# mratsim/constantine

Hardware: NVIDIA H100
Metric: bls12_381_g1_msm_throughput (higher is better)
Workload: dtype u32

## Files before the change

constantine_b200/csrc/msm_affine.cuh:

```cuda
#pragma once
#include "ec.cuh"
#include "field_inv.cuh"

namespace b200 {

constexpr int AFF_MAX_LEVELS = 8;
constexpr uint32_t AFF_NONE = 0xFFFFFFFFu;

static __global__ void k_bucket_bounds(const uint32_t* __restrict__ keys, size_t n, uint32_t no_key, uint32_t* head, uint32_t* tail) {
  size_t q = (size_t)blockIdx.x * blockDim.x + threadIdx.x;
  if (q >= n) return;
  const uint32_t key = keys[q];
  if (key >= no_key) return;
  if (q == 0 || keys[q - 1] != key) head[key] = (uint32_t)q;
  if (q + 1 == n || keys[q + 1] != key) tail[key] = (uint32_t)(q + 1);
}

constexpr int SCAN_THREADS = 256, SCAN_PER_THREAD = 4, SCAN_ITEMS = SCAN_THREADS * SCAN_PER_THREAD;

B200_DEV uint32_t block_exclusive_scan(uint32_t v, uint32_t& total, uint32_t* smem ) {
  const unsigned lane = threadIdx.x & 31u, warp = threadIdx.x >> 5;
  uint32_t inc = v;
#pragma unroll
  for (int d = 1; d < 32; d <<= 1) {
    uint32_t t = __shfl_up_sync(0xFFFFFFFFu, inc, d);
    if (lane >= (unsigned)d) inc += t;
  }
  __syncthreads();
  if (lane == 31u) smem[warp] = inc;
  __syncthreads();
  uint32_t base = 0, tot = 0;
#pragma unroll
  for (int w = 0; w < SCAN_THREADS / 32; w++) {
    const uint32_t s = smem[w];
    if ((unsigned)w < warp) base += s;
    tot += s;
  }
  total = tot;
  return base + inc - v;
}

B200_DEV uint32_t level_count(uint32_t n, int r) { return (n + (1u << r) - 1u) >> r; }

static __global__ void __launch_bounds__(SCAN_THREADS) k_level_blocksums(const uint32_t* __restrict__ head, const uint32_t* __restrict__ tail,
                                                                          uint32_t nb, int L, uint32_t nblk, uint32_t* blocksum ) {
  __shared__ uint32_t sm[SCAN_THREADS / 32 + 1];
  const uint32_t b0 = blockIdx.x * SCAN_ITEMS + threadIdx.x * SCAN_PER_THREAD;
  uint32_t cnt[SCAN_PER_THREAD];
#pragma unroll
  for (int k = 0; k < SCAN_PER_THREAD; k++) cnt[k] = (b0 + k < nb) ? tail[b0 + k] - head[b0 + k] : 0u;
  for (int r = 0; r <= L; r++) {
    uint32_t s = 0;
#pragma unroll
    for (int k = 0; k < SCAN_PER_THREAD; k++) s += level_count(cnt[k], r);
    uint32_t tot;
    block_exclusive_scan(s, tot, sm);
    if (threadIdx.x == 0) blocksum[(size_t)r * nblk + blockIdx.x] = tot;
  }
}

static __global__ void __launch_bounds__(SCAN_THREADS) k_level_scan(uint32_t* blocksum, uint32_t nblk, int L, uint32_t nb, uint32_t* off) {
  __shared__ uint32_t sm[SCAN_THREADS / 32 + 1];
  for (int r = 0; r <= L; r++) {
    uint32_t carry = 0;
    for (uint32_t base = 0; base < nblk; base += SCAN_THREADS) {
      const uint32_t i = base + threadIdx.x;
      const uint32_t v = (i < nblk) ? blocksum[(size_t)r * nblk + i] : 0u;
      uint32_t tot;
      const uint32_t ex = block_exclusive_scan(v, tot, sm);
      if (i < nblk) blocksum[(size_t)r * nblk + i] = carry + ex;
      carry += tot;
    }
    if (threadIdx.x == 0) off[(size_t)r * (nb + 1) + nb] = carry;
  }
}

static __global__ void __launch_bounds__(SCAN_THREADS) k_level_offsets(const uint32_t* __restrict__ head, const uint32_t* __restrict__ tail,
                                                                        uint32_t nb, int L, uint32_t nblk, const uint32_t* __restrict__ blocksum,
                                                                        uint32_t* off) {
  __shared__ uint32_t sm[SCAN_THREADS / 32 + 1];
  const uint32_t b0 = blockIdx.x * SCAN_ITEMS + threadIdx.x * SCAN_PER_THREAD;
  uint32_t cnt[SCAN_PER_THREAD];
#pragma unroll
  for (int k = 0; k < SCAN_PER_THREAD; k++) cnt[k] = (b0 + k < nb) ? tail[b0 + k] - head[b0 + k] : 0u;
  for (int r = 0; r <= L; r++) {
    uint32_t c[SCAN_PER_THREAD], s = 0;
#pragma unroll
    for (int k = 0; k < SCAN_PER_THREAD; k++) { c[k] = level_count(cnt[k], r); s += c[k]; }
    uint32_t tot;
    uint32_t ex = block_exclusive_scan(s, tot, sm) + blocksum[(size_t)r * nblk + blockIdx.x];
#pragma unroll
    for (int k = 0; k < SCAN_PER_THREAD; k++) {
      if (b0 + k < nb) off[(size_t)r * (nb + 1) + b0 + k] = ex;
      ex += c[k];
    }
  }
}

struct AffinePlan {
  uint2* plan0;
  uint32_t* plan[AFF_MAX_LEVELS];
  uint32_t* surv_keys;
  uint32_t* surv_vals;
};

static __global__ void k_affine_plan(const uint32_t* __restrict__ keys, const uint32_t* __restrict__ vals, size_t n, uint32_t no_key,
                                     const uint32_t* __restrict__ head, const uint32_t* __restrict__ tail,
                                     const uint32_t* __restrict__ off, uint32_t nb, int L, AffinePlan P) {
  size_t q = (size_t)blockIdx.x * blockDim.x + threadIdx.x;
  if (q >= n) return;
  const uint32_t b = keys[q];
  if (b >= no_key) return;
  const uint32_t h = head[b], i = (uint32_t)q - h, cnt = tail[b] - h;
  const size_t stride = (size_t)nb + 1;
  for (int r = 0; r < L; r++) {
    if (i & ((2u << r) - 1u)) break;
    const uint32_t p = off[(size_t)(r + 1) * stride + b] + (i >> (r + 1));
    const uint32_t s = i >> r;
    const bool has2 = s + 1u < level_count(cnt, r);
    if (r == 0) P.plan0[p] = make_uint2(vals[q], has2 ? vals[q + 1] : AFF_NONE);
    else P.plan[r][p] = (off[(size_t)r * stride + b] + s) | (has2 ? 0x80000000u : 0u);
  }
  if ((i & ((1u << L) - 1u)) == 0u) {
    const uint32_t ps = off[(size_t)L * stride + b] + (i >> L);
    P.surv_keys[ps] = b;
    P.surv_vals[ps] = ps;
  }
}

template <class T>
B200_DEV Aff<T> load_affine_rw(const uint32_t* base, size_t idx) {
  const uint32_t* p = base + idx * (2 * T::WORDS);
  Aff<T> a;
  load_words_rw(a.x, p);
  load_words_rw(a.y, p + T::WORDS);
  return a;
}
template <class T>
B200_DEV void store_affine(uint32_t* base, size_t idx, const Aff<T>& a) {
  uint32_t* p = base + idx * (2 * T::WORDS);
  store_words(p, a.x);
  store_words(p + T::WORDS, a.y);
}

template <class T>
B200_DEV void scratch_store(uint4* scratch, size_t threads, size_t tid, uint32_t j, const T& v) {
  constexpr int V = T::WORDS / 4;
#pragma unroll
  for (int k = 0; k < V; k++) {
    uint4 w;
    w.x = v.word(4 * k + 0); w.y = v.word(4 * k + 1); w.z = v.word(4 * k + 2); w.w = v.word(4 * k + 3);
    scratch[((size_t)j * V + k) * threads + tid] = w;
  }
}
template <class T>
B200_DEV T scratch_load(const uint4* scratch, size_t threads, size_t tid, uint32_t j) {
  constexpr int V = T::WORDS / 4;
  T v;
#pragma unroll
  for (int k = 0; k < V; k++) {
    const uint4 w = scratch[((size_t)j * V + k) * threads + tid];
    v.set_word(4 * k + 0, w.x); v.set_word(4 * k + 1, w.y); v.set_word(4 * k + 2, w.z); v.set_word(4 * k + 3, w.w);
  }
  return v;
}

constexpr int PART_TILE = 1024, PART_THREADS = 256, PART_MAX = 8;

B200_DEV uint32_t pair_chunk(const uint2 task, uint32_t n_points, uint32_t P) {
  uint32_t idx = task.x & 0x7FFFFFFFu;
  if (task.y != AFF_NONE) { const uint32_t j = task.y & 0x7FFFFFFFu; if (j > idx) idx = j; }
  uint32_t q = (uint32_t)(((unsigned long long)idx * P) / n_points);
  return q < P ? q : P - 1u;
}

static __global__ void __launch_bounds__(PART_THREADS) k_part_count(const uint2* __restrict__ plan0, const uint32_t* __restrict__ total_ptr,
                                                                    uint32_t n_points, uint32_t P, uint32_t nblk, uint32_t* counts) {
  __shared__ uint32_t sm[PART_MAX];
  if (threadIdx.x < PART_MAX) sm[threadIdx.x] = 0;
  __syncthreads();
  const uint32_t total = *total_ptr;
  const uint32_t base = blockIdx.x * PART_TILE;
  uint32_t local[PART_MAX];
#pragma unroll
  for (int q = 0; q < PART_MAX; q++) local[q] = 0;
  for (uint32_t i = threadIdx.x; i < PART_TILE; i += PART_THREADS) {
    const uint32_t p = base + i;
    if (p < total) {
      const uint32_t q = pair_chunk(plan0[p], n_points, P);
#pragma unroll
      for (int k = 0; k < PART_MAX; k++) local[k] += (q == (uint32_t)k) ? 1u : 0u;
    }
  }
#pragma unroll
  for (int q = 0; q < PART_MAX; q++) {
    uint32_t v = local[q];
    for (int d = 16; d >= 1; d >>= 1) v += __shfl_xor_sync(0xFFFFFFFFu, v, d);
    if ((threadIdx.x & 31u) == 0 && v) atomicAdd(&sm[q], v);
  }
  __syncthreads();
  if (threadIdx.x < P) counts[threadIdx.x * nblk + blockIdx.x] = sm[threadIdx.x];
}

static __global__ void __launch_bounds__(SCAN_THREADS) k_part_scan(uint32_t* counts, uint32_t P, uint32_t nblk, uint32_t* starts) {
  __shared__ uint32_t sm[SCAN_THREADS / 32 + 1];
  uint32_t carry = 0;
  const uint32_t len = P * nblk;
  for (uint32_t base = 0; base < len; base += SCAN_THREADS) {
    const uint32_t i = base + threadIdx.x;
    const uint32_t v = (i < len) ? counts[i] : 0u;
    uint32_t tot;
    const uint32_t ex = block_exclusive_scan(v, tot, sm);
    if (i < len) {
      counts[i] = carry + ex;
      if (i % nblk == 0) starts[i / nblk] = carry + ex;
    }
    carry += tot;
  }
  if (threadIdx.x == 0) starts[P] = carry;
}

static __global__ void __launch_bounds__(PART_THREADS) k_part_scatter(const uint2* __restrict__ plan0, const uint32_t* __restrict__ total_ptr,
                                                                      uint32_t n_points, uint32_t P, uint32_t nblk,
                                                                      const uint32_t* __restrict__ offsets, uint32_t* perm) {
  __shared__ uint32_t warp_cnt[PART_THREADS / 32][PART_MAX];
  __shared__ uint32_t run_base[PART_MAX];
  const uint32_t total = *total_ptr;
  const unsigned lane = threadIdx.x & 31u, warp = threadIdx.x >> 5;
  if (threadIdx.x < PART_MAX) run_base[threadIdx.x] = (threadIdx.x < P) ? offsets[threadIdx.x * nblk + blockIdx.x] : 0u;
  __syncthreads();
  for (uint32_t round = 0; round < PART_TILE / PART_THREADS; round++) {
    const uint32_t p = blockIdx.x * PART_TILE + round * PART_THREADS + threadIdx.x;
    const bool live = p < total;
    const uint32_t q = live ? pair_chunk(plan0[p], n_points, P) : 0xFFFFFFFFu;
    uint32_t my_rank = 0;
    for (uint32_t k = 0; k < P; k++) {
      const unsigned m = __ballot_sync(0xFFFFFFFFu, q == k);
      if (q == k) my_rank = __popc(m & ((1u << lane) - 1u));
      if (lane == 0) warp_cnt[warp][k] = __popc(m);
    }
    __syncthreads();
    if (live) {
      uint32_t before = 0;
      for (unsigned w = 0; w < warp; w++) before += warp_cnt[w][q];
      perm[run_base[q] + before + my_rank] = p;
    }
    __syncthreads();
    if (threadIdx.x < P) {
      uint32_t tot = 0;
      for (unsigned w = 0; w < PART_THREADS / 32; w++) tot += warp_cnt[w][threadIdx.x];
      run_base[threadIdx.x] += tot;
    }
    __syncthreads();
  }
}

enum PairKind { PAIR_COPY1 = 0, PAIR_COPY2 = 1, PAIR_INF = 2, PAIR_ADD = 3, PAIR_DBL = 4 };

struct PairTask {
  uint32_t a, b;
};
template <bool FIRST>
B200_DEV PairTask load_task(const void* plan, size_t p) {
  PairTask t;
  if constexpr (FIRST) {
    const uint2 v = reinterpret_cast<const uint2*>(plan)[p];
    t.a = v.x; t.b = v.y;
  } else {
    const uint32_t v = reinterpret_cast<const uint32_t*>(plan)[p];
    t.a = v & 0x7FFFFFFFu;
    t.b = (v >> 31) ? t.a + 1u : AFF_NONE;
  }
  return t;
}
template <class T, bool FIRST>
B200_DEV T load_x(const uint32_t* src, uint32_t ref) {
  T x;
  if constexpr (FIRST) load_words(x, src + (size_t)(ref & 0x7FFFFFFFu) * (2 * T::WORDS));
  else load_words_rw(x, src + (size_t)ref * (2 * T::WORDS));
  return x;
}
template <class T, bool FIRST>
B200_DEV T load_y(const uint32_t* src, uint32_t ref, bool& is_inf_if_x_zero) {
  T y;
  if constexpr (FIRST) {
    load_words(y, src + (size_t)(ref & 0x7FFFFFFFu) * (2 * T::WORDS) + T::WORDS);
    is_inf_if_x_zero = y.is_zero();
    y.cneg((ref >> 31) != 0);
  } else {
    load_words_rw(y, src + (size_t)ref * (2 * T::WORDS) + T::WORDS);
    is_inf_if_x_zero = y.is_zero();
  }
  return y;
}

template <class T>
B200_DEV int classify_pair(bool single, const T& x1, const T& y1, bool inf1, const T& x2, const T& y2, bool inf2, T& den) {
  if (single) return PAIR_COPY1;
  if (inf1) return PAIR_COPY2;
  if (inf2) return PAIR_COPY1;
  den = x2 - x1;
  if (!den.is_zero()) return PAIR_ADD;
  if (!(y1 == y2) || y1.is_zero()) return PAIR_INF;
  den = y1.dbl();
  return PAIR_DBL;
}

#ifndef B200_AFF_THREADS
#define B200_AFF_THREADS 128
#endif
#ifndef B200_AFF_MIN_BLOCKS
#define B200_AFF_MIN_BLOCKS 4
#endif

B200_DEV void prefetch_l2(const void* p) { asm volatile("prefetch.global.L2 [%0];" ::"l"(p)); }
B200_DEV void prefetch_span(const void* p, int bytes) {
  prefetch_l2(p);
  prefetch_l2((const char*)p + bytes - 1);
}
template <class T, bool FIRST>
B200_DEV void prefetch_point(const uint32_t* src, uint32_t ref) {
  const uint32_t idx = FIRST ? (ref & 0x7FFFFFFFu) : ref;
  prefetch_span(src + (size_t)idx * (2 * T::WORDS), 2 * T::WORDS * 4);
}

template <class T, bool FIRST>
__global__ void __launch_bounds__(B200_AFF_THREADS, (T::WORDS <= 12) ? B200_AFF_MIN_BLOCKS : 1)
k_affine_pairs(const void* __restrict__ plan, const uint32_t* __restrict__ total_ptr, const uint32_t* src, uint32_t* dst, uint4* scratch,
               const uint32_t* __restrict__ perm = nullptr, const uint32_t* __restrict__ range = nullptr) {
  const size_t threads = (size_t)gridDim.x * blockDim.x;
  const size_t tid = (size_t)blockIdx.x * blockDim.x + threadIdx.x;
  const uint32_t range_begin = range ? range[0] : 0u;
  const uint32_t total = range ? range[1] - range[0] : *total_ptr;
  if (perm) perm += range_begin;
  const uint32_t M = (uint32_t)(((size_t)total + threads - 1) / threads);
  const unsigned lane = threadIdx.x & 31u;
  const size_t warp_base = (tid - lane) * (size_t)M;
  if (warp_base >= total) return;
  uint32_t cnt = 0;
  {
    const size_t first = warp_base + lane;
    if (first < total) {
      const size_t left = (size_t)total - first;
      cnt = (uint32_t)((left + 31) / 32);
      if (cnt > M) cnt = M;
    }
  }
  T run = T::one();
  {
    auto slot_of = [&](size_t t) -> size_t { return perm ? (size_t)perm[t] : t; };
    PairTask t_next = cnt ? load_task<FIRST>(plan, slot_of(warp_base + lane)) : PairTask{0u, AFF_NONE};
    T x1n = T::zero(), x2n = T::zero();
    if (cnt) {
      x1n = load_x<T, FIRST>(src, t_next.a);
      if (t_next.b != AFF_NONE) x2n = load_x<T, FIRST>(src, t_next.b);
    }
#pragma unroll 1
    for (uint32_t j = 0; j < cnt; j++) {
      const PairTask t = t_next;
      const T x1 = x1n, x2 = x2n;
      if (j + 1 < cnt) {
        t_next = load_task<FIRST>(plan, slot_of(warp_base + lane + 32u * (size_t)(j + 1)));
        x1n = load_x<T, FIRST>(src, t_next.a);
        if (t_next.b != AFF_NONE) x2n = load_x<T, FIRST>(src, t_next.b);
      }
      const bool single = t.b == AFF_NONE;
      T den = x2 - x1;
      bool contributes = !single;
      if (!single && (den.is_zero() || x1.is_zero() || x2.is_zero())) {
        bool z1, z2;
        const T y1 = load_y<T, FIRST>(src, t.a, z1), y2 = load_y<T, FIRST>(src, t.b, z2);
        const int kind = classify_pair(false, x1, y1, z1 && x1.is_zero(), x2, y2, z2 && x2.is_zero(), den);
        contributes = kind >= PAIR_ADD;
      }
      if (contributes) run = run.mul_u(den);
      scratch_store(scratch, threads, tid, j, run);
    }
  }
  T inv = fe_inverse(run);
  auto slot_of2 = [&](size_t t) -> size_t { return perm ? (size_t)perm[t] : t; };
  size_t p_prev = cnt ? slot_of2(warp_base + lane + 32u * (size_t)(cnt - 1)) : 0;
  PairTask t_prev = cnt ? load_task<FIRST>(plan, p_prev) : PairTask{0u, AFF_NONE};
#pragma unroll 1
  for (uint32_t jj = cnt; jj > 0; jj--) {
    const uint32_t j = jj - 1;
    const size_t p = p_prev;
    const PairTask t = t_prev;
    if (j > 0) {
      p_prev = slot_of2(warp_base + lane + 32u * (size_t)(j - 1));
      t_prev = load_task<FIRST>(plan, p_prev);
      prefetch_point<T, FIRST>(src, t_prev.a);
      if (t_prev.b != AFF_NONE) prefetch_point<T, FIRST>(src, t_prev.b);
      if (j > 1) {
        constexpr int V = T::WORDS / 4;
#pragma unroll
        for (int k = 0; k < V; k++) prefetch_l2(scratch + ((size_t)(j - 2) * V + k) * threads + tid);
      }
    }
    const bool single = t.b == AFF_NONE;
    Aff<T> P1, P2;
    bool z1 = false, z2 = false;
    P1.x = load_x<T, FIRST>(src, t.a);
    P1.y = load_y<T, FIRST>(src, t.a, z1);
    if (!single) {
      P2.x = load_x<T, FIRST>(src, t.b);
      P2.y = load_y<T, FIRST>(src, t.b, z2);
    } else {
      P2.x = T::zero(); P2.y = T::zero();
    }
    T den;
    const int kind = classify_pair(single, P1.x, P1.y, z1 && P1.x.is_zero(), P2.x, P2.y, z2 && P2.x.is_zero(), den);
    Aff<T> R;
    if (kind < PAIR_ADD) {
      if (kind == PAIR_COPY1) R = P1;
      else if (kind == PAIR_COPY2) R = P2;
      else { R.x = T::zero(); R.y = T::zero(); }
    } else {
      T inv_den = inv;
      if (j > 0) inv_den = inv.mul_u(scratch_load<T>(scratch, threads, tid, j - 1));
      inv = inv.mul_u(den);
      T num;
      if (kind == PAIR_ADD) num = P2.y - P1.y;
      else { const T xx = P1.x.sqr(); num = xx.dbl() + xx; }
      const T lam = num.mul_u(inv_den);
      R.x = lam.sqr_u() - P1.x - P2.x;
      R.y = lam.mul_u(P1.x - R.x) - P1.y;
    }
    store_affine(dst, p, R);
  }
}

#ifndef B200_AFF_WS_CONSUMERS
#define B200_AFF_WS_CONSUMERS 8
#endif
#ifndef B200_AFF_WS_STAGES
#define B200_AFF_WS_STAGES 2
#endif
constexpr int AFF_WS_CONSUMERS = B200_AFF_WS_CONSUMERS;
constexpr int AFF_WS_THREADS = 32 * (AFF_WS_CONSUMERS + 1);

template <class T>
struct AffRing {
  static constexpr bool USED = T::WORDS <= 12;
  static constexpr int V = T::WORDS / 4;
  static constexpr int S2 = B200_AFF_WS_STAGES;
  static constexpr int ROWS = S2 * 5 * V;
  static constexpr int S1 = ROWS / (2 * V);
  static constexpr size_t BYTES = (size_t)AFF_WS_CONSUMERS * ROWS * 32 * 16;
};

B200_DEV uint32_t smem_addr(const void* p) { return (uint32_t)__cvta_generic_to_shared(p); }
B200_DEV void mbar_init(uint64_t* b, uint32_t count) { asm volatile("mbarrier.init.shared::cta.b64 [%0], %1;" ::"r"(smem_addr(b)), "r"(count) : "memory"); }
B200_DEV void mbar_arrive(uint64_t* b) { asm volatile("mbarrier.arrive.shared::cta.b64 _, [%0];" ::"r"(smem_addr(b)) : "memory"); }
B200_DEV void mbar_wait(uint64_t* b, uint32_t parity) {
  asm volatile(
      "{\n\t.reg .pred P1;\n"
      "WAIT:\n\t"
      "mbarrier.try_wait.parity.shared::cta.b64 P1, [%0], %1;\n\t"
      "@!P1 bra WAIT;\n\t}" ::"r"(smem_addr(b)),
      "r"(parity)
      : "memory");
}
B200_DEV void cp_async_arrive(uint64_t* b) { asm volatile("cp.async.mbarrier.arrive.noinc.shared::cta.b64 [%0];" ::"r"(smem_addr(b)) : "memory"); }
B200_DEV void cp_async16(void* s, const void* g) { asm volatile("cp.async.cg.shared.global [%0], [%1], 16;" ::"r"(smem_addr(s)), "l"(g) : "memory"); }

template <class T>
B200_DEV void ring_fetch(uint4* ring, int row, unsigned lane, const uint32_t* g) {
#pragma unroll
  for (int k = 0; k < T::WORDS / 4; k++) cp_async16(ring + (row + k) * 32 + lane, g + 4 * k);
}
template <class T>
B200_DEV T ring_load(const uint4* ring, int row, unsigned lane) {
  T v;
#pragma unroll
  for (int k = 0; k < T::WORDS / 4; k++) {
    const uint4 w = ring[(row + k) * 32 + lane];
    v.set_word(4 * k + 0, w.x); v.set_word(4 * k + 1, w.y); v.set_word(4 * k + 2, w.z); v.set_word(4 * k + 3, w.w);
  }
  return v;
}

template <class T, bool FIRST>
__global__ void __launch_bounds__(AFF_WS_THREADS, 1)
k_affine_pairs_ws(const void* __restrict__ plan, const uint32_t* __restrict__ total_ptr, const uint32_t* src, uint32_t* dst, uint4* scratch,
                  const uint32_t* __restrict__ perm = nullptr, const uint32_t* __restrict__ range = nullptr) {
  using RG = AffRing<T>;
  constexpr int V = RG::V, NC = AFF_WS_CONSUMERS, S1 = RG::S1, S2 = RG::S2;
  extern __shared__ __align__(16) unsigned char aff_ring_raw[];
  __shared__ uint64_t full1[NC][S1], empty1[NC][S1], full2[NC][S2], empty2[NC][S2], drained[NC];
  __shared__ uint32_t s_task[NC][S1][3][32];
  const unsigned lane = threadIdx.x & 31u, warp = threadIdx.x >> 5;
  if (threadIdx.x == 0) {
    for (int w = 0; w < NC; w++) {
      for (int s = 0; s < S1; s++) { mbar_init(&full1[w][s], 64); mbar_init(&empty1[w][s], 32); }
      for (int s = 0; s < S2; s++) { mbar_init(&full2[w][s], 64); mbar_init(&empty2[w][s], 32); }
      mbar_init(&drained[w], 32);
    }
  }
  __syncthreads();
  const size_t threads = (size_t)gridDim.x * NC * 32;
  const uint32_t range_begin = range ? range[0] : 0u;
  const uint32_t total = range ? range[1] - range[0] : *total_ptr;
  if (perm) perm += range_begin;
  const uint32_t M = (uint32_t)(((size_t)total + threads - 1) / threads);
  auto count_of = [&](size_t tid) -> uint32_t {
    const size_t first = (tid & ~(size_t)31) * M + (tid & 31u);
    if (first >= total) return 0u;
    const uint32_t c = (uint32_t)(((size_t)total - first + 31) / 32);
    return c < M ? c : M;
  };
  auto slot_at = [&](size_t tid, uint32_t j) -> size_t {
    const size_t t = (tid & ~(size_t)31) * M + (tid & 31u) + 32u * (size_t)j;
    return perm ? (size_t)perm[t] : t;
  };
  uint4* const ring_base = reinterpret_cast<uint4*>(aff_ring_raw);

  if (warp == NC) {
    uint32_t n[NC], cnt[NC];
#pragma unroll
    for (int w = 0; w < NC; w++) {
      const size_t tid = ((size_t)blockIdx.x * NC + w) * 32 + lane;
      n[w] = count_of(tid - lane);
      cnt[w] = count_of(tid);
    }
    auto tid_of = [&](int w) { return ((size_t)blockIdx.x * NC + w) * 32 + lane; };
    auto src_of = [&](uint32_t ref) { return src + (size_t)(FIRST ? (ref & 0x7FFFFFFFu) : ref) * (2 * T::WORDS); };
    uint32_t ta[NC], tb[NC], tp[NC];
    auto fetch_task = [&](int w, uint32_t j) {
      const size_t p = slot_at(tid_of(w), j);
      const PairTask t = load_task<FIRST>(plan, p);
      ta[w] = t.a; tb[w] = t.b; tp[w] = (uint32_t)p;
    };
#pragma unroll
    for (int w = 0; w < NC; w++) if (cnt[w]) fetch_task(w, 0);
#pragma unroll 1
    for (uint32_t j = 0; j < n[0]; j++) {
      uint32_t ca[NC], cb[NC];
#pragma unroll
      for (int w = 0; w < NC; w++) { ca[w] = ta[w]; cb[w] = tb[w]; }
#pragma unroll
      for (int w = 0; w < NC; w++) if (j + 1 < cnt[w]) fetch_task(w, j + 1);
#pragma unroll
      for (int w = 0; w < NC; w++) {
        if (j >= n[w]) continue;
        const int s = (int)(j % S1);
        mbar_wait(&empty1[w][s], ((j / S1) & 1u) ^ 1u);
        uint4* ring = ring_base + (size_t)w * RG::ROWS * 32;
        if (j < cnt[w]) {
          s_task[w][s][0][lane] = ca[w];
          s_task[w][s][1][lane] = cb[w];
          ring_fetch<T>(ring, s * 2 * V, lane, src_of(ca[w]));
          if (cb[w] != AFF_NONE) ring_fetch<T>(ring, s * 2 * V + V, lane, src_of(cb[w]));
        }
        cp_async_arrive(&full1[w][s]);
        mbar_arrive(&full1[w][s]);
      }
    }
#pragma unroll
    for (int w = 0; w < NC; w++) if (n[w] && n[w] - 1 < cnt[w]) fetch_task(w, n[w] - 1);
#pragma unroll 1
    for (uint32_t jj = 0; jj < n[0]; jj++) {
      uint32_t ca[NC], cb[NC], cp[NC];
#pragma unroll
      for (int w = 0; w < NC; w++) { ca[w] = ta[w]; cb[w] = tb[w]; cp[w] = tp[w]; }
#pragma unroll
      for (int w = 0; w < NC; w++) if (jj + 1 < n[w] && n[w] - 2 - jj < cnt[w]) fetch_task(w, n[w] - 2 - jj);
#pragma unroll
      for (int w = 0; w < NC; w++) {
        if (jj >= n[w]) continue;
        if (jj == 0) mbar_wait(&drained[w], 0);
        const uint32_t j = n[w] - 1 - jj;
        const int s = (int)(jj % S2);
        mbar_wait(&empty2[w][s], ((jj / S2) & 1u) ^ 1u);
        uint4* ring = ring_base + (size_t)w * RG::ROWS * 32;
        if (j < cnt[w]) {
          s_task[w][s][0][lane] = ca[w];
          s_task[w][s][1][lane] = cb[w];
          s_task[w][s][2][lane] = cp[w];
          const int row = s * 5 * V;
          ring_fetch<T>(ring, row, lane, src_of(ca[w]));
          ring_fetch<T>(ring, row + V, lane, src_of(ca[w]) + T::WORDS);
          if (cb[w] != AFF_NONE) {
            ring_fetch<T>(ring, row + 2 * V, lane, src_of(cb[w]));
            ring_fetch<T>(ring, row + 3 * V, lane, src_of(cb[w]) + T::WORDS);
          }
          if (j > 0) {
#pragma unroll
            for (int k = 0; k < V; k++)
              cp_async16(ring + (row + 4 * V + k) * 32 + lane, scratch + ((size_t)(j - 1) * V + k) * threads + tid_of(w));
          }
        }
        cp_async_arrive(&full2[w][s]);
        mbar_arrive(&full2[w][s]);
      }
    }
    asm volatile("cp.async.wait_all;" ::: "memory");
    return;
  }

  const size_t tid = ((size_t)blockIdx.x * NC + warp) * 32 + lane;
  const uint32_t n = count_of(tid - lane), cnt = count_of(tid);
  if (n == 0) return;
  const uint4* ring = ring_base + (size_t)warp * RG::ROWS * 32;
  T run = T::one();
#pragma unroll 1
  for (uint32_t j = 0; j < n; j++) {
    const int s = (int)(j % S1);
    mbar_wait(&full1[warp][s], (j / S1) & 1u);
    const uint32_t a = s_task[warp][s][0][lane], b = s_task[warp][s][1][lane];
    const T x1 = ring_load<T>(ring, s * 2 * V, lane), x2 = ring_load<T>(ring, s * 2 * V + V, lane);
    mbar_arrive(&empty1[warp][s]);
    if (j >= cnt) continue;
    const bool single = b == AFF_NONE;
    T den = x2 - x1;
    bool contributes = !single;
    if (!single && (den.is_zero() || x1.is_zero() || x2.is_zero())) {
      bool z1, z2;
      const T y1 = load_y<T, FIRST>(src, a, z1), y2 = load_y<T, FIRST>(src, b, z2);
      const int kind = classify_pair(false, x1, y1, z1 && x1.is_zero(), x2, y2, z2 && x2.is_zero(), den);
      contributes = kind >= PAIR_ADD;
    }
    if (contributes) run = run.mul_u(den);
    scratch_store(scratch, threads, tid, j, run);
  }
  mbar_arrive(&drained[warp]);
  T inv = fe_inverse(run);
#pragma unroll 1
  for (uint32_t jj = 0; jj < n; jj++) {
    const uint32_t j = n - 1 - jj;
    const int s = (int)(jj % S2);
    mbar_wait(&full2[warp][s], (jj / S2) & 1u);
    const int row = s * 5 * V;
    const uint32_t a = s_task[warp][s][0][lane], b = s_task[warp][s][1][lane], p = s_task[warp][s][2][lane];
    const bool single = b == AFF_NONE;
    Aff<T> P1, P2;
    P1.x = ring_load<T>(ring, row, lane);
    P1.y = ring_load<T>(ring, row + V, lane);
    P2.x = single ? T::zero() : ring_load<T>(ring, row + 2 * V, lane);
    P2.y = single ? T::zero() : ring_load<T>(ring, row + 3 * V, lane);
    const T pre = ring_load<T>(ring, row + 4 * V, lane);
    mbar_arrive(&empty2[warp][s]);
    if (j >= cnt) continue;
    const bool z1 = P1.y.is_zero(), z2 = P2.y.is_zero();
    if constexpr (FIRST) {
      P1.y.cneg((a >> 31) != 0);
      if (!single) P2.y.cneg((b >> 31) != 0);
    }
    T den;
    const int kind = classify_pair(single, P1.x, P1.y, z1 && P1.x.is_zero(), P2.x, P2.y, z2 && P2.x.is_zero(), den);
    Aff<T> R;
    if (kind < PAIR_ADD) {
      if (kind == PAIR_COPY1) R = P1;
      else if (kind == PAIR_COPY2) R = P2;
      else { R.x = T::zero(); R.y = T::zero(); }
    } else {
      T inv_den = inv;
      if (j > 0) inv_den = inv.mul_u(pre);
      inv = inv.mul_u(den);
      T num;
      if (kind == PAIR_ADD) num = P2.y - P1.y;
      else { const T xx = P1.x.sqr(); num = xx.dbl() + xx; }
      const T lam = num.mul_u(inv_den);
      R.x = lam.sqr_u() - P1.x - P2.x;
      R.y = lam.mul_u(P1.x - R.x) - P1.y;
    }
    store_affine(dst, p, R);
  }
}

template <class T>
constexpr int affine_pairs_slot_threads() { return AffRing<T>::USED ? 32 * AFF_WS_CONSUMERS : B200_AFF_THREADS; }

template <class T>
cudaError_t affine_pairs_blocks_per_sm(int* bps) {
  int b1 = 0, b2 = 0;
  cudaError_t e;
  if constexpr (AffRing<T>::USED) {
    constexpr int bytes = (int)AffRing<T>::BYTES;
    if ((e = cudaFuncSetAttribute(k_affine_pairs_ws<T, true>, cudaFuncAttributeMaxDynamicSharedMemorySize, bytes)) != cudaSuccess) return e;
    if ((e = cudaFuncSetAttribute(k_affine_pairs_ws<T, false>, cudaFuncAttributeMaxDynamicSharedMemorySize, bytes)) != cudaSuccess) return e;
    if ((e = cudaOccupancyMaxActiveBlocksPerMultiprocessor(&b1, k_affine_pairs_ws<T, true>, AFF_WS_THREADS, bytes)) != cudaSuccess) return e;
    if ((e = cudaOccupancyMaxActiveBlocksPerMultiprocessor(&b2, k_affine_pairs_ws<T, false>, AFF_WS_THREADS, bytes)) != cudaSuccess) return e;
  } else {
    if ((e = cudaOccupancyMaxActiveBlocksPerMultiprocessor(&b1, k_affine_pairs<T, true>, B200_AFF_THREADS, 0)) != cudaSuccess) return e;
    if ((e = cudaOccupancyMaxActiveBlocksPerMultiprocessor(&b2, k_affine_pairs<T, false>, B200_AFF_THREADS, 0)) != cudaSuccess) return e;
  }
  *bps = b2 < b1 ? b2 : b1;
  return cudaSuccess;
}

template <class T, bool FIRST>
void launch_affine_pairs(unsigned grid, cudaStream_t s, const void* plan, const uint32_t* total_ptr, const uint32_t* src, uint32_t* dst, uint4* scratch,
                         const uint32_t* perm = nullptr, const uint32_t* range = nullptr) {
  if constexpr (AffRing<T>::USED)
    k_affine_pairs_ws<T, FIRST><<<grid, AFF_WS_THREADS, AffRing<T>::BYTES, s>>>(plan, total_ptr, src, dst, scratch, perm, range);
  else
    k_affine_pairs<T, FIRST><<<grid, B200_AFF_THREADS, 0, s>>>(plan, total_ptr, src, dst, scratch, perm, range);
}

}
```

Measured before the change: 108.5.

## Split warp-specialized affine kernel into four producers and twelve consumers with setmaxnreg

Restructures the warp-specialized affine pair kernel from eight consumer warps fed by one producer warp into twelve consumers fed by four producer warps, each producer serving three consumers. setmaxnreg moves registers from the producers (32) to the consumers (160) so the consumers' field arithmetic has more register room. Task prefetch is interleaved with issuing fetches per consumer. The plan kernel is also rewritten to compute the level count with ffs and to preload offsets and values before the loop. The change depends on setmaxnreg behavior and carries a risk of spills if consumers need more than 160 registers.

```diff
diff --git a/constantine_b200/csrc/msm_affine.cuh b/constantine_b200/csrc/msm_affine.cuh
--- a/constantine_b200/csrc/msm_affine.cuh
+++ b/constantine_b200/csrc/msm_affine.cuh
@@ -113,16 +113,27 @@
   if (b >= no_key) return;
   const uint32_t h = head[b], i = (uint32_t)q - h, cnt = tail[b] - h;
   const size_t stride = (size_t)nb + 1;
-  for (int r = 0; r < L; r++) {
-    if (i & ((2u << r) - 1u)) break;
-    const uint32_t p = off[(size_t)(r + 1) * stride + b] + (i >> (r + 1));
+  const int lv = i ? min(__ffs((int)i) - 1, L) : L;
+  uint32_t o[AFF_MAX_LEVELS + 1];
+#pragma unroll
+  for (int r = 1; r <= AFF_MAX_LEVELS; r++) if (r <= lv) o[r] = off[(size_t)r * stride + b];
+  const uint32_t o_surv = lv == L ? off[(size_t)L * stride + b] : 0u;
+  uint32_t v0 = 0, v1 = AFF_NONE;
+  if (lv >= 1) {
+    v0 = vals[q];
+    if (i + 1u < cnt) v1 = vals[q + 1];
+  }
+#pragma unroll
+  for (int r = 0; r < AFF_MAX_LEVELS; r++) {
+    if (r >= lv) break;
+    const uint32_t p = o[r + 1] + (i >> (r + 1));
     const uint32_t s = i >> r;
     const bool has2 = s + 1u < level_count(cnt, r);
-    if (r == 0) P.plan0[p] = make_uint2(vals[q], has2 ? vals[q + 1] : AFF_NONE);
-    else P.plan[r][p] = (off[(size_t)r * stride + b] + s) | (has2 ? 0x80000000u : 0u);
-  }
-  if ((i & ((1u << L) - 1u)) == 0u) {
-    const uint32_t ps = off[(size_t)L * stride + b] + (i >> L);
+    if (r == 0) P.plan0[p] = make_uint2(v0, v1);
+    else P.plan[r][p] = (o[r] + s) | (has2 ? 0x80000000u : 0u);
+  }
+  if (lv == L) {
+    const uint32_t ps = o_surv + (i >> L);
     P.surv_keys[ps] = b;
     P.surv_vals[ps] = ps;
   }
@@ -430,14 +441,18 @@
   }
 }
 
-#ifndef B200_AFF_WS_CONSUMERS
-#define B200_AFF_WS_CONSUMERS 8
-#endif
 #ifndef B200_AFF_WS_STAGES
 #define B200_AFF_WS_STAGES 2
 #endif
-constexpr int AFF_WS_CONSUMERS = B200_AFF_WS_CONSUMERS;
-constexpr int AFF_WS_THREADS = 32 * (AFF_WS_CONSUMERS + 1);
+constexpr int AFF_WS_CONSUMERS = 12;
+constexpr int AFF_WS_PRODUCERS = 4;
+constexpr int AFF_WS_FEEDS = AFF_WS_CONSUMERS / AFF_WS_PRODUCERS;
+constexpr int AFF_WS_THREADS = 32 * (AFF_WS_CONSUMERS + AFF_WS_PRODUCERS);
+constexpr int AFF_WS_CONSUMER_REGS = 160, AFF_WS_PRODUCER_REGS = 32;
+static_assert(AFF_WS_CONSUMERS % 4 == 0 && AFF_WS_PRODUCERS == 4, "setmaxnreg acts on whole warpgroups");
+static_assert(32 * (AFF_WS_CONSUMERS * AFF_WS_CONSUMER_REGS + AFF_WS_PRODUCERS * AFF_WS_PRODUCER_REGS) == 65536 &&
+                  65536 / AFF_WS_THREADS == 128,
+              "the register split must fill exactly the registers the launch gives the block");
 
 template <class T>
 struct AffRing {
@@ -463,6 +478,10 @@
 }
 B200_DEV void cp_async_arrive(uint64_t* b) { asm volatile("cp.async.mbarrier.arrive.noinc.shared::cta.b64 [%0];" ::"r"(smem_addr(b)) : "memory"); }
 B200_DEV void cp_async16(void* s, const void* g) { asm volatile("cp.async.cg.shared.global [%0], [%1], 16;" ::"r"(smem_addr(s)), "l"(g) : "memory"); }
+template <int R>
+B200_DEV void setmaxnreg_inc() { asm volatile("setmaxnreg.inc.sync.aligned.u32 %0;" ::"n"(R)); }
+template <int R>
+B200_DEV void setmaxnreg_dec() { asm volatile("setmaxnreg.dec.sync.aligned.u32 %0;" ::"n"(R)); }
 
 template <class T>
 B200_DEV void ring_fetch(uint4* ring, int row, unsigned lane, const uint32_t* g) {
@@ -485,7 +504,7 @@
 k_affine_pairs_ws(const void* __restrict__ plan, const uint32_t* __restrict__ total_ptr, const uint32_t* src, uint32_t* dst, uint4* scratch,
                   const uint32_t* __restrict__ perm = nullptr, const uint32_t* __restrict__ range = nullptr) {
   using RG = AffRing<T>;
-  constexpr int V = RG::V, NC = AFF_WS_CONSUMERS, S1 = RG::S1, S2 = RG::S2;
+  constexpr int V = RG::V, NC = AFF_WS_CONSUMERS, F = AFF_WS_FEEDS, S1 = RG::S1, S2 = RG::S2;
   extern __shared__ __align__(16) unsigned char aff_ring_raw[];
   __shared__ uint64_t full1[NC][S1], empty1[NC][S1], full2[NC][S2], empty2[NC][S2], drained[NC];
   __shared__ uint32_t s_task[NC][S1][3][32];
@@ -509,95 +528,90 @@
     const uint32_t c = (uint32_t)(((size_t)total - first + 31) / 32);
     return c < M ? c : M;
   };
-  auto slot_at = [&](size_t tid, uint32_t j) -> size_t {
-    const size_t t = (tid & ~(size_t)31) * M + (tid & 31u) + 32u * (size_t)j;
-    return perm ? (size_t)perm[t] : t;
-  };
   uint4* const ring_base = reinterpret_cast<uint4*>(aff_ring_raw);
 
-  if (warp == NC) {
-    uint32_t n[NC], cnt[NC];
-#pragma unroll
-    for (int w = 0; w < NC; w++) {
-      const size_t tid = ((size_t)blockIdx.x * NC + w) * 32 + lane;
-      n[w] = count_of(tid - lane);
-      cnt[w] = count_of(tid);
-    }
-    auto tid_of = [&](int w) { return ((size_t)blockIdx.x * NC + w) * 32 + lane; };
+  if (warp >= NC) {
+    setmaxnreg_dec<AFF_WS_PRODUCER_REGS>();
+    const int w0 = (int)(warp - NC) * F;
+    const uint32_t tid0 = ((uint32_t)blockIdx.x * NC + w0) * 32 + lane;
+    auto first = [&](int i) { return (tid0 + 32u * i - lane) * M + lane; };
+    auto has_slot = [&](int i, uint32_t j) { return j < M && first(i) + 32u * j < total; };
+    auto rounds = [&](int i) -> uint32_t {
+      const uint32_t b = first(i) - lane;
+      return b < total ? min((total - b - 1) / 32 + 1, M) : 0u;
+    };
     auto src_of = [&](uint32_t ref) { return src + (size_t)(FIRST ? (ref & 0x7FFFFFFFu) : ref) * (2 * T::WORDS); };
-    uint32_t ta[NC], tb[NC], tp[NC];
-    auto fetch_task = [&](int w, uint32_t j) {
-      const size_t p = slot_at(tid_of(w), j);
-      const PairTask t = load_task<FIRST>(plan, p);
-      ta[w] = t.a; tb[w] = t.b; tp[w] = (uint32_t)p;
+    auto slot = [&](int i, uint32_t j) { const uint32_t t = first(i) + 32u * j; return perm ? perm[t] : t; };
+    uint32_t ta[F], tb[F];
+    auto fetch_task = [&](int i, uint32_t j) {
+      const PairTask tk = load_task<FIRST>(plan, slot(i, j));
+      ta[i] = tk.a; tb[i] = tk.b;
     };
 #pragma unroll
-    for (int w = 0; w < NC; w++) if (cnt[w]) fetch_task(w, 0);
+    for (int i = 0; i < F; i++) if (has_slot(i, 0)) fetch_task(i, 0);
 #pragma unroll 1
-    for (uint32_t j = 0; j < n[0]; j++) {
-      uint32_t ca[NC], cb[NC];
-#pragma unroll
-      for (int w = 0; w < NC; w++) { ca[w] = ta[w]; cb[w] = tb[w]; }
-#pragma unroll
-      for (int w = 0; w < NC; w++) if (j + 1 < cnt[w]) fetch_task(w, j + 1);
-#pragma unroll
-      for (int w = 0; w < NC; w++) {
-        if (j >= n[w]) continue;
-        const int s = (int)(j % S1);
+    for (uint32_t j = 0; j < rounds(0); j++) {
+#pragma unroll
+      for (int i = 0; i < F; i++) {
+        if (j >= rounds(i)) continue;
+        const int w = w0 + i, s = (int)(j % S1);
         mbar_wait(&empty1[w][s], ((j / S1) & 1u) ^ 1u);
         uint4* ring = ring_base + (size_t)w * RG::ROWS * 32;
-        if (j < cnt[w]) {
-          s_task[w][s][0][lane] = ca[w];
-          s_task[w][s][1][lane] = cb[w];
-          ring_fetch<T>(ring, s * 2 * V, lane, src_of(ca[w]));
-          if (cb[w] != AFF_NONE) ring_fetch<T>(ring, s * 2 * V + V, lane, src_of(cb[w]));
+        if (has_slot(i, j)) {
+          s_task[w][s][0][lane] = ta[i];
+          s_task[w][s][1][lane] = tb[i];
+          ring_fetch<T>(ring, s * 2 * V, lane, src_of(ta[i]));
+          if (tb[i] != AFF_NONE) ring_fetch<T>(ring, s * 2 * V + V, lane, src_of(tb[i]));
         }
         cp_async_arrive(&full1[w][s]);
         mbar_arrive(&full1[w][s]);
+        if (has_slot(i, j + 1)) fetch_task(i, j + 1);
       }
     }
 #pragma unroll
-    for (int w = 0; w < NC; w++) if (n[w] && n[w] - 1 < cnt[w]) fetch_task(w, n[w] - 1);
+    for (int i = 0; i < F; i++) {
+      const uint32_t r = rounds(i);
+      if (r && has_slot(i, r - 1)) fetch_task(i, r - 1);
+    }
 #pragma unroll 1
-    for (uint32_t jj = 0; jj < n[0]; jj++) {
-      uint32_t ca[NC], cb[NC], cp[NC];
-#pragma unroll
-      for (int w = 0; w < NC; w++) { ca[w] = ta[w]; cb[w] = tb[w]; cp[w] = tp[w]; }
-#pragma unroll
-      for (int w = 0; w < NC; w++) if (jj + 1 < n[w] && n[w] - 2 - jj < cnt[w]) fetch_task(w, n[w] - 2 - jj);
-#pragma unroll
-      for (int w = 0; w < NC; w++) {
-        if (jj >= n[w]) continue;
+    for (uint32_t jj = 0; jj < rounds(0); jj++) {
+#pragma unroll
+      for (int i = 0; i < F; i++) {
+        const uint32_t r = rounds(i);
+        if (jj >= r) continue;
+        const int w = w0 + i;
         if (jj == 0) mbar_wait(&drained[w], 0);
-        const uint32_t j = n[w] - 1 - jj;
+        const uint32_t j = r - 1 - jj;
         const int s = (int)(jj % S2);
         mbar_wait(&empty2[w][s], ((jj / S2) & 1u) ^ 1u);
         uint4* ring = ring_base + (size_t)w * RG::ROWS * 32;
-        if (j < cnt[w]) {
-          s_task[w][s][0][lane] = ca[w];
-          s_task[w][s][1][lane] = cb[w];
-          s_task[w][s][2][lane] = cp[w];
+        if (has_slot(i, j)) {
+          s_task[w][s][0][lane] = ta[i];
+          s_task[w][s][1][lane] = tb[i];
+          s_task[w][s][2][lane] = slot(i, j);
           const int row = s * 5 * V;
-          ring_fetch<T>(ring, row, lane, src_of(ca[w]));
-          ring_fetch<T>(ring, row + V, lane, src_of(ca[w]) + T::WORDS);
-          if (cb[w] != AFF_NONE) {
-            ring_fetch<T>(ring, row + 2 * V, lane, src_of(cb[w]));
-            ring_fetch<T>(ring, row + 3 * V, lane, src_of(cb[w]) + T::WORDS);
+          ring_fetch<T>(ring, row, lane, src_of(ta[i]));
+          ring_fetch<T>(ring, row + V, lane, src_of(ta[i]) + T::WORDS);
+          if (tb[i] != AFF_NONE) {
+            ring_fetch<T>(ring, row + 2 * V, lane, src_of(tb[i]));
+            ring_fetch<T>(ring, row + 3 * V, lane, src_of(tb[i]) + T::WORDS);
           }
           if (j > 0) {
 #pragma unroll
             for (int k = 0; k < V; k++)
-              cp_async16(ring + (row + 4 * V + k) * 32 + lane, scratch + ((size_t)(j - 1) * V + k) * threads + tid_of(w));
+              cp_async16(ring + (row + 4 * V + k) * 32 + lane, scratch + ((size_t)(j - 1) * V + k) * threads + (tid0 + 32u * i));
           }
         }
         cp_async_arrive(&full2[w][s]);
         mbar_arrive(&full2[w][s]);
+        if (j > 0 && has_slot(i, j - 1)) fetch_task(i, j - 1);
       }
     }
     asm volatile("cp.async.wait_all;" ::: "memory");
     return;
   }
 
+  setmaxnreg_inc<AFF_WS_CONSUMER_REGS>();
   const size_t tid = ((size_t)blockIdx.x * NC + warp) * 32 + lane;
   const uint32_t n = count_of(tid - lane), cnt = count_of(tid);
   if (n == 0) return;
```

After: 113.0 (median of 6 runs). 1.04x the previous value.
